# JustinPrivitera/Real_Time_Ray_Tracer

Hardware: AMD Instinct MI355X
Metric: Mrays/s + ms/frame at 3840x2160, 16 AO samples, 64 spheres; 1/2/4/8 GPU (higher is better)
Workload: dtype f32

## Files before the change

__graft_entry__.py:

```python
from __future__ import annotations

import os
import subprocess
import sys
from pathlib import Path

ROOT = Path(__file__).resolve().parent


def build() -> None:
    env = dict(os.environ)
    env.setdefault("PYTORCH_ROCM_ARCH", "gfx950")
    jobs = str(min(16, os.cpu_count() or 1))
    subprocess.run(["make", "-j", jobs, "lib", "headless", "oracle", "b1sort0"], cwd=ROOT, check=True, env=env)
    if str(ROOT) not in sys.path:
        sys.path.insert(0, str(ROOT))
    import real_time_ray_tracer_amd as rt

    rt.load()


def smoke() -> None:
    if str(ROOT) not in sys.path:
        sys.path.insert(0, str(ROOT))
    import numpy as np

    import oracle
    import real_time_ray_tracer_amd as rt

    W, H, spp = 64, 48, 4
    h = rt.Header.synthetic(16, spp, 1234, rt.aspect_for(W, H))
    r = rt.Renderer(W, H, h.S, h.AA, device=0)
    ho = h.copy()
    s = rt.SSBO(ho, W, H)
    d = oracle.dims(W, H, h.S, h.AA)
    img = np.zeros((H, W, 4), np.float32)
    fg = fo = 0
    for k in range(3):
        h.fill_rand_buffer(7000 + k)
        h.set_mode(fg, h.num_objects)
        r.upload_header(h)
        fg = r.dispatch(rt.host._lib.RT_MODE_AO_PP, fg)
        s.set_header(h)
        fo = oracle.dispatch(s.data, d, 1, fo, img)
    g = r.download()
    r.close()
    ok = np.abs(g.image - img) <= 1e-4 * np.maximum(np.abs(g.image), np.abs(img)) + 1e-6
    if not ok.all() or fg != fo:
        raise RuntimeError(f"smoke: {int((~ok).sum())} image values differ from the oracle")
    if not np.array_equal(g.depth.view(np.uint32), s.depth.view(np.uint32)):
        raise RuntimeError("smoke: depth g-buffer differs from the oracle")
    print(f"smoke ok: {W}x{H} mode 1, 3 frames, image mean {img[..., :3].mean():.4f}")


if __name__ == "__main__":
    build()
    if len(sys.argv) > 1 and sys.argv[1] == "smoke":
        smoke()
```

real_time_ray_tracer_amd/csrc/rt_kernels_impl.h:

```cpp
#pragma once
#include <hip/hip_runtime.h>

#include "rt_device.h"
#include "rt_kernels.h"

namespace rt {

namespace {

constexpr int kBlock = 256;
constexpr float kGamma = 1.0f / 2.2f;

__device__ __forceinline__ void stage_shapes(const FrameParams& P, float4* lds) {
  const int n = P.nobj;
  for (int k = threadIdx.x; k < 4 * n; k += blockDim.x) {
    int tab = k / n, i = k - tab * n;
    lds[k] = P.shapes[(size_t)tab * P.S + i];
  }
}

__device__ __forceinline__ f3 primary_dir(const FrameParams& P, float hp, float vp) {
  f3 a = mk(P.lx + hp * P.hx, P.ly + hp * P.hy, P.lz + hp * P.hz);
  return normalize(mk(a.x + vp * P.vx, a.y + vp * P.vy, a.z + vp * P.vz));
}
// ... 506 lines not shown
  float t;
  int ind;
  if (ALLSPH) {
    const ConeF cone = wave_tile_cone<BWX, BWY>(P, bx, by);
    ind = closest_hit_cone<PL>(P, geo, n, cone, cam, dir, 0.0f, t, pre0);
  } else {
    ind = closest_hit<ALLSPH>(geo, geo2, n, cam, dir, 0.0f, t);
  }
  count_work(P, active, y, 1u, active && ind != -1 ? 1u : 0u);
  const bool need = active && ind != -1;
  bool lit_w = true;
  if (ALLSPH) lit_w = shadow_lit_cone<PL>(P, geo, n, light, cam + t * dir, need, pre0);
  if (!active) return;
  float r, g, b;
  if (ind == -1) {
    r = P.bg.x; g = P.bg.y; b = P.bg.z;
  } else {
    f3 curr = cam + t * dir;
    bool lit = ALLSPH ? lit_w : shadow_lit<ALLSPH>(geo, geo2, n, light, curr);
    int id = (ALLSPH && !PL) ? SHAPE_SPHERE : __float_as_int(geo2[ind].w);
    f3 nn = shape_normal(tab[ind], id, curr);
    float4 c = col[ind];
    if (lit) {
      f3 l = normalize(light - curr);
      float spec = pow500(gclamp(dot(normalize(l - dir), nn), 0.0f, 1.0f));
      float k = gclamp(dot(nn, l), 0.06f, 1.0f);
      r = c.x * k + spec; g = c.y * k + spec; b = c.z * k + spec;
    } else {
      r = c.x * 0.06f; g = c.y * 0.06f; b = c.z * 0.06f;
    }
  }
  store_color(P, fd.out_pix, fd.image, x, y, gamma_out(0.0f + r, 0.0f + g, 0.0f + b));
}

#ifndef RT_TAB_LDS_MAX
#define RT_TAB_LDS_MAX 128
#endif
constexpr int kTabLdsMax = RT_TAB_LDS_MAX;
__device__ __forceinline__ void stage_tables(const FrameParams& P, float4* lds) {
  const int n = P.nobj;
  stage_shapes(P, lds);
  for (int k = threadIdx.x; k < n; k += blockDim.x) lds[4 * n + k] = P.sph[k];
}

template <bool ALLSPH, bool PL = false, bool LT = false, bool MF = true>
__global__ __launch_bounds__(kBlock) void phong_kernel(const float4* __restrict__ gsph, const float4* __restrict__ gshp,
                                                       FrameParams P) {
  extern __shared__ float4 lds[];
  if (!ALLSPH || LT) {
    if (LT) stage_tables(P, lds);
    else stage_shapes(P, lds);
    __syncthreads();
  }
  if constexpr (!MF) {
    const float4 g0 = gsph[threadIdx.x & 63];
    phong_tile<ALLSPH, PL, LT>(P, lds, blockIdx.x, blockIdx.y, frame_dst<false>(P, 0), gsph, gshp,
                               (ALLSPH && !LT) ? &g0 : nullptr);
    return;
  }
  int j0;
  const int nj = block_frames<kPhongFramesPerBlock>(P, j0);
#pragma unroll 1
  for (int j = 0; j < nj; ++j)
    phong_tile<ALLSPH, PL, LT>(P, lds, blockIdx.x, blockIdx.y, frame_dst(P, j0 + j), gsph, gshp);
}

template <bool PL>
__device__ __forceinline__ void bounce_round(const FrameParams& P, const float4* __restrict__ geo, int n, f3 light,
                                             bool live, f3 pos, f3 dir, int* perm, float& t_out, int& ind_out,
                                             bool& lit_out) {
  const unsigned long long lm = __ballot(live);
  const int L = __popcll(lm);
  const int lane = threadIdx.x & 63;
  if (L > 32) {
    float t = -1.0f;
    int ind = -1;
    bool lit = true;
    if (live) {
      ind = closest_hit_pf(geo, n, pos, dir, 0.001f, t);
      if (PL) plane_pass(P, pos, dir, 0.001f, t, ind);
      if (ind != -1) lit = shadow_lit_sph<PL>(P, geo, n, light, pos + t * dir);
    }
    t_out = t;
    ind_out = ind;
    lit_out = lit;
    return;
  }
  int c = 0;
  while ((1 << c) < L) ++c;
  const int G = 64 >> c;
  const int rk = __builtin_amdgcn_mbcnt_hi((unsigned)(lm >> 32), __builtin_amdgcn_mbcnt_lo((unsigned)lm, 0u));
  if (live) perm[rk] = lane;
  __builtin_amdgcn_wave_barrier();
  const int g = lane / G, pl = lane - g * G;
  const bool act = g < L;
  const int owner = act ? perm[g] : lane;
  __builtin_amdgcn_wave_barrier();
  const f3 o = mk(__shfl(pos.x, owner), __shfl(pos.y, owner), __shfl(pos.z, owner));
  const f3 d = mk(__shfl(dir.x, owner), __shfl(dir.y, owner), __shfl(dir.z, owner));
  float t = -1.0f;
  int ind = -1;
  if (act)
    for (int i = pl; i < n; i += G) sphere_candidate(o, d, geo[i], i, 0.001f, t, ind);
  for (int m = 1; m < G; m <<= 1) {
    const float tb = __shfl_xor(t, m);
    const int ib = __shfl_xor(ind, m);
    const bool take = ib >= 0 && (ind < 0 || tb < t || (tb == t && ib < ind));
    t = take ? tb : t;
    ind = take ? ib : ind;
  }
  if (PL && act) plane_pass(P, o, d, 0.001f, t, ind);
  bool occ = false;
  if (act && ind != -1) {
    const f3 curr = o + t * d;
    const f3 lv = light - curr;
    const f3 l = normalize(lv);
    const float len = sqrtf(dot(lv, lv));
    const f3 np = curr + 0.01f * l;
    const double dlen = (double)len;
    const ShadowBounds sb = shadow_bounds(l, len);
    if (PL)
      for (int k = pl; k < P.nplanes && !occ; k += G)
        occ = shadow_occludes(plane_eval(np, l, P.planes[2 * k], P.planes[2 * k + 1]), l, dlen, sb);
    for (int i = pl; i < n && !occ; i += G) occ = shadow_occludes(sphere_eval_shadow(np, l, geo[i]), l, dlen, sb);
  }
  unsigned oc = occ ? 1u : 0u;
  for (int m = 1; m < G; m <<= 1) oc |= (unsigned)__shfl_xor((int)oc, m);
  const int src = live ? rk * G : lane;
  t_out = __shfl(t, src);
  ind_out = __shfl(ind, src);
  lit_out = __shfl((int)oc, src) == 0;
}

template <bool ALLSPH, bool PL, bool LT, int ABL = 0, int BWX = 2, int BWY = 2>
__device__ __forceinline__ void hybrid_tile(const FrameParams& P, const float4* lds, int* perm, int bx, int by,
                                            const FrameDst& fd, const float4* __restrict__ gsph,
                                            const float4* __restrict__ gshp, const float4* pre0 = nullptr) {
  const int n = P.nobj;
  const float4* tab = (ALLSPH && !LT) ? gshp : lds;
  const float4* geo = (ALLSPH && !LT) ? gsph : (ALLSPH ? lds + 4 * n : lds);
  const int stride = (ALLSPH && !LT) ? P.S : n;
  const float4 *geo2 = tab + stride, *col = tab + 2 * stride, *aux = tab + 3 * stride;
  int x, y;
  tile_xy<BWX, BWY>(x, y, P.trace_row0, bx, by);
  const bool active = x < P.W && y < P.trace_row0 + P.trace_rows;
  const f3 light = fd.light;
  const unsigned long long tstart = ABL == 7 ? __builtin_amdgcn_s_memrealtime() : 0;
  f3 pos = mk(P.cx, P.cy, P.cz);
  f3 dir = primary_dir(P, div_rn_by((float)x, P.fW, P.inv_W), div_rn_by((float)y, P.fH, P.inv_H));
  float arefl = 0.0f;
  float rr = 0, rg = 0, rb = 0;
  float c = 0.0f;
  unsigned nseg = 0, nshadow = 0;
  auto segment = [&](int seg, float t, int ind, bool lit) -> bool {
    ++nseg;
    nshadow += ind == -1 ? 0u : 1u;
    float ar, ag, ab;
    bool stop;
    if (ind == -1) {
      ar = P.bg.x; ag = P.bg.y; ab = P.bg.z;
      stop = true;
    } else {
      float4 att = ABL == 9 ? make_float4(0.5f, 0.5f, 0.5f, 0.0f) : col[ind];
      f3 curr = pos + t * dir;
      int id = (ALLSPH && !PL) ? SHAPE_SPHERE : __float_as_int(geo2[ind].w);
      f3 nn = ABL == 9 ? normalize(curr) : shape_normal(tab[ind], id, curr);
      if (lit) {
        f3 l = normalize(light - curr);
        float spec = pow500(gclamp(dot(normalize(l - dir), nn), 0.0f, 1.0f));
        float k = gclamp(dot(nn, l), 0.06f, 1.0f);
        ar = att.x * k + spec; ag = att.y * k + spec; ab = att.z * k + spec;
      } else {
        ar = att.x * 0.06f; ag = att.y * 0.06f; ab = att.z * 0.06f;
      }
      float refl = ABL == 9 ? 0.0f : 1.0f - aux[ind].y;
      if (refl < 0.001f) {
        stop = true;
      } else {
        stop = false;
        float dn = dot(dir, nn);
        dir = normalize(mk(dir.x - 2.0f * (dn * nn.x), dir.y - 2.0f * (dn * nn.y),
                           dir.z - 2.0f * (dn * nn.z)));
        pos = curr;
        arefl = refl;
      }
    }
    if (seg == 0) {
      c = arefl;
      rr = ar; rg = ag; rb = ab;
    } else {
      float den = 1.0f + c;
      rr = (rr + c * ar) / den;
      rg = (rg + c * ag) / den;
      rb = (rb + c * ab) / den;
      c = c * arefl;
    }
    return stop;
  };
  if (ALLSPH) {
    float t0 = -1.0f;
    int ind0 = -1;
    bool lit0 = true;
    const ConeF cone = wave_tile_cone<BWX, BWY>(P, bx, by);
    if (ABL != 2) ind0 = closest_hit_cone<PL, ABL == 3>(P, geo, n, cone, pos, dir, 0.001f, t0, pre0);
    if (ABL == 0 || ABL >= 4) lit0 = shadow_lit_cone<PL>(P, geo, n, light, pos + t0 * dir, active && ind0 != -1, pre0);
    bool live = active && !segment(0, t0, ind0, lit0);
    int rounds = 0;
    for (int seg = 1; seg < ((ABL == 5 || ABL == 9) ? 1 : P.D); ++seg) {
      if (__ballot(live) == 0) break;
      ++rounds;
      float t;
      int ind;
      bool lit = true;
      if (ABL == 6) {
        if (live) {
          ind = closest_hit_pf(geo, n, pos, dir, 0.001f, t);
          if (PL) plane_pass(P, pos, dir, 0.001f, t, ind);
          if (ind != -1) lit = shadow_lit_sph<PL>(P, geo, n, light, pos + t * dir);
        }
      } else {
        bounce_round<PL>(P, geo, n, light, live, pos, dir, perm, t, ind, lit);
      }
      if (live) live = !segment(seg, t, ind, lit);
    }
    if (P.tile_cost && (threadIdx.x & 63) == 0)
      P.tile_cost[((unsigned)by * gridDim.x + (unsigned)bx) * (BWX * BWY) + (threadIdx.x >> 6)] = (unsigned)rounds;
  } else {
    for (int seg = 0; active && seg < P.D; ++seg) {
      float t;
      const int ind = closest_hit<ALLSPH>(geo, geo2, n, pos, dir, 0.001f, t);
      const bool lit = ind == -1 || shadow_lit<ALLSPH>(geo, geo2, n, light, pos + t * dir);
      if (segment(seg, t, ind, lit)) break;
    }
  }
  count_work(P, active, y, nseg, nshadow);
  if (active) store_color(P, fd.out_pix, fd.image, x, y, gamma_out(0.0f + rr, 0.0f + rg, 0.0f + rb));
  if (ABL == 7) {
    const unsigned mx = wave_max(active ? nseg : 0u);
    const unsigned long long tend = __builtin_amdgcn_s_memrealtime();
    if ((threadIdx.x & 63) == 0 && active)
      P.out_pix[(size_t)(y - P.band_row0) * P.W + x] =
          make_float4(__uint_as_float((unsigned)tstart), __uint_as_float((unsigned)tend), __uint_as_float(mx),
                      __uint_as_float((unsigned)(tstart >> 32)));
  }
}

template <bool ALLSPH, bool PL = false, bool LT = false, int ABL = 0, int BWX = 2, int BWY = 2, bool MF = true>
__global__ __launch_bounds__(64 * BWX * BWY) void hybrid_kernel(const unsigned* __restrict__ tord,
                                                                const float4* __restrict__ gsph,
                                                                const float4* __restrict__ gshp, unsigned gx,
                                                                FrameParams P) {
  extern __shared__ float4 lds[];
  __shared__ int hperm[64 * BWX * BWY];
  if (!ALLSPH || LT) {
    if (LT) stage_tables(P, lds);
    else stage_shapes(P, lds);
    __syncthreads();
  }
  if constexpr (kHybridTilesPerBlock == 2) {
    const unsigned gx = gridDim.x, gy = (unsigned)(P.trace_rows + 8 * BWY - 1) / (8 * BWY), n = gx * gy;
    const unsigned b = blockIdx.x + blockIdx.y * gx;
#pragma unroll 1
    for (int t = 0; t < 2; ++t) {
      const unsigned u = t == 0 ? b : n - 1 - b;
      if (b > n - 1 - b || (t == 1 && u == b)) break;
      unsigned bx = u % gx, by = u / gx;
      if (tord) {
        const unsigned v = tord[u];
        bx = v & 0xffffu;
        by = v >> 16;
      }
      hybrid_tile<ALLSPH, PL, LT, ABL, BWX, BWY>(P, lds, hperm + 64 * (threadIdx.x >> 6), bx, by, frame_dst(P, blockIdx.z), gsph, gshp);
    }
  } else if constexpr (kHybridTilesPerBlock > 1) {
#pragma unroll 1
    for (int t = 0; t < kHybridTilesPerBlock; ++t)
      hybrid_tile<ALLSPH, PL, LT, ABL, BWX, BWY>(P, lds, hperm + 64 * (threadIdx.x >> 6), blockIdx.x,
                                                 blockIdx.y * kHybridTilesPerBlock + t, frame_dst(P, blockIdx.z), gsph, gshp);
  } else if constexpr (kHybridFramesPerBlock == 1) {
    const bool pre = !MF && ALLSPH && !LT;
    float4 g0;
    if (pre) g0 = gsph[threadIdx.x & 63];
    unsigned bx = blockIdx.x, by = blockIdx.y;
    if (tord) {
      const unsigned t = tord[blockIdx.x + blockIdx.y * gx];
      bx = t & 0xffffu;
      by = t >> 16;
    }
    hybrid_tile<ALLSPH, PL, LT, ABL, BWX, BWY>(P, lds, hperm + 64 * (threadIdx.x >> 6), bx, by,
                                               frame_dst<MF>(P, blockIdx.z), gsph, gshp, pre ? &g0 : nullptr);
  } else {
    int j0;
    const int nj = block_frames<kHybridFramesPerBlock>(P, j0);
#pragma unroll 1
    for (int j = 0; j < nj; ++j)
      hybrid_tile<ALLSPH, PL, LT, ABL, BWX, BWY>(P, lds, hperm + 64 * (threadIdx.x >> 6), blockIdx.x, blockIdx.y,
                                                 frame_dst(P, j0 + j), gsph, gshp);
  }
}

enum { PRIM_HIT = 0, PRIM_MISS = 1, PRIM_EMISSIVE = 2 };

struct BatchLds {
  int prec, sres, pstop, pkind, perm, order, cmask, rls, geol, total;
};
__host__ __device__ constexpr BatchLds batch_lds(int spp, int pool, int ntail, bool rls_lds = true, bool sort = false) {
  const int TP = pool / spp > 0 ? pool / spp : 1, NS = TP * spp;
  BatchLds L{};
  L.prec = 0;
  L.sres = 16 * TP;
  L.pstop = L.sres + 12 * NS;
  L.pkind = L.pstop + 4 * TP;
  L.perm = L.pkind + 4 * ((TP + 1) & ~1);
  L.order = L.perm + 256;
  L.cmask = (L.order + (sort ? pool : 0) + 7) & ~7;
  L.rls = (L.cmask + 8 * 32 + 15) & ~15;
  L.geol = L.rls + (rls_lds ? 32 * spp : 0);
  L.total = L.geol + 16 * ntail;
  return L;
}

#ifndef RT_AO_MINW
#define RT_AO_MINW 7
#endif
#ifndef RT_PT_WIDE
#define RT_PT_WIDE 1
#endif
#ifndef RT_B1_DEFER
#define RT_B1_DEFER 1
#endif
#ifndef RT_B1_PRIO
#define RT_B1_PRIO 1
#endif
#ifndef RT_START_PRIO
#define RT_START_PRIO 1
#endif
#ifndef RT_B1_CREAD
#define RT_B1_CREAD 1
#endif
#ifndef RT_B1_SORT
#define RT_B1_SORT 1
#endif
constexpr int kAoMinWaves = RT_AO_MINW;
template <int MINW, bool LAZY = true, int POOL = kPool, int ABL = 0, bool TAIL = false, bool B1 = false,
          int SPPC = 0, bool PT = false, bool CNT = true, bool PL = false, bool MF = false, bool CL = true, int DC = 0,
          bool CLON = false, bool PTW = false, bool SORT = false>
__global__ __launch_bounds__(64, MINW) void ao_batch_kernel(FrameParams P, const float4* __restrict__ geo) {
  if (RT_START_PRIO) __builtin_amdgcn_s_setprio(1);
  unsigned long long* const cnts = CNT ? P.counters : nullptr;
  unsigned long long* const rowc = CNT ? P.row_counters : nullptr;
  extern __shared__ float4 lds[];
  const int spp = SPPC ? SPPC : P.spp, W = P.W, D = DC ? DC : P.D, nobj = P.nobj;
  const bool use_cl = CL && (CLON || P.ncl > 0);
  const int fj = MF ? (int)blockIdx.y : 0;
  const int fslot = MF ? (P.mf_slot0 + fj) % P.F : 0;
  float4* const f_nrm = MF ? (float4*)P.hist_nrm[fslot] : P.nrm;
  float4* const f_dep = MF ? (float4*)P.hist_dep[fslot] : P.dep;
  const float4* const f_nrm_prev = MF ? f_nrm : P.nrm_prev;
  const float4* const f_dep_prev = MF ? f_dep : P.dep_prev;
  float4* const f_out = MF ? (float4*)P.hist_pix[fslot] : P.out_pix;
  float4* const f_img = MF ? (fj == P.mf_n - 1 ? P.image : nullptr) : P.image;
  const float4* const f_rb = MF ? P.mf_rb + (size_t)fj * 2 * spp : P.rb;
  const int TP = POOL / spp > 0 ? POOL / spp : 1;
  const int lane = threadIdx.x;
  const int NS = TP * spp;
  static_assert(!SORT || (LAZY && POOL % 64 == 0 && POOL <= 256), "SORT: hemi is read back from LDS; items are bytes");
  const BatchLds LO = batch_lds(spp, POOL, 0, !PTW, SORT);
  char* lbase = (char*)lds;
  float4* prec = (float4*)(lbase + LO.prec);
  float* sres = (float*)(lbase + LO.sres);
  int* pstop = (int*)(lbase + LO.pstop);
  int* pkind = (int*)(lbase + LO.pkind);
  int* perm = (int*)(lbase + LO.perm);
  unsigned char* order = (unsigned char*)(lbase + LO.order);
  unsigned long long* cmask = (unsigned long long*)(lbase + LO.cmask);
  float4* rls = (float4*)(lbase + LO.rls);
  if (!PTW)
    for (int k = lane; k < 2 * spp; k += 64) rls[k] = f_rb[k];
  for (int k = lane; k < TP; k += 64) pstop[k] = -1;
  float4* geol = (float4*)(lbase + LO.geol);
  constexpr bool tail_lds = TAIL && PT && !PTW;
  const bool tail_ok = TAIL;
  const float4* const tgeo = tail_lds ? geol : geo;
  const bool pt_ok = PT && B1 && (tail_lds || PTW);
  bool geol_valid = false;
  if (tail_lds && !pt_ok) {
    for (int k = lane; k < nobj; k += 64) geol[k] = geo[k];
    geol_valid = true;
  }
  const float4* const clus = geo + (size_t)3 * P.S;
  const unsigned long long* const clm = (const unsigned long long*)(geo + (size_t)3 * P.S + kMaxClusters);
  auto col_at = [&](int ind) -> float4 {
    int o = ind - P.S;
    asm("" : "+v"(o));
    return geo[o - P.S];
  };
  auto aux_at = [&](int ind) -> float4 {
    int o = ind - P.S;
    asm("" : "+v"(o));
    return geo[o];
  };

  const long long npix = (long long)P.trace_rows * W;
  unsigned pb = blockIdx.x;
  if (P.pool_rot > 0) {
    const unsigned Q = (unsigned)P.pool_rot, r = pb / Q;
    if ((r + 1) * Q <= gridDim.x) {
      unsigned c = pb - r * Q + r % Q;
      c = c >= Q ? c - Q : c;
      pb = r * Q + c;
    }
  }
  const long long p0 = (long long)pb * TP;
  const int np = (int)(npix - p0 < TP ? npix - p0 : TP);
  const int total = np * spp;

  unsigned long long tsec[8] = {0, 0, 0, 0, 0, 0, 0, 0};
  constexpr bool kLaps = ABL == 3 || ABL == 6 || ABL == 8;
  unsigned long long tmark = kLaps ? __builtin_amdgcn_s_memtime() : 0;
  auto lap = [&](int k) {
    if (kLaps) {
      unsigned long long now = __builtin_amdgcn_s_memtime();
      tsec[k] += now - tmark;
      tmark = now;
    }
  };
  const int yf = P.trace_row0 + (int)(p0 / W), xf = (int)(p0 % W);
  auto pool_xy = [&](int lp, int& x, int& y) {
    int xi = xf + lp;
    y = yf;
    if (xi >= W) {
      int q = (int)((unsigned)xi / (unsigned)W);
      y += q;
      xi -= q * W;
    }
    x = xi;
  };
  const int yl = P.trace_row0 + (int)((p0 + np - 1) / W), xl = (int)((p0 + np - 1) % W);
  int ncull = 0;
  const int nwords = (nobj + 63) >> 6;
  unsigned long long pmask = 0;
  {
    const ConeF cone = pool_cone_f(P, yf == yl ? xf : 0, yf == yl ? xl : W - 1, yf, yl);
    for (int w = 0; w < nwords; ++w) {
      int i = (w << 6) + lane;
      bool keep = i < nobj && !cone_misses_f(cone, geo[i], P.cx, P.cy, P.cz);
      if (PL) keep = keep && geo[i].x == geo[i].x;
      unsigned long long m = __ballot(keep);
      ncull += __popcll(m);
      if (lane == 0) cmask[w] = m;
    }
    if (PL) {
      pmask = plane_cone_mask(P, cone, mk(P.cx, P.cy, P.cz));
      ncull += __popcll(pmask) + (P.nplanes > 64 ? P.nplanes - 64 : 0);
    }
  }
  __syncthreads();
  lap(0);
  if (RT_START_PRIO) __builtin_amdgcn_s_setprio(0);

  if (LAZY && ncull == 0) {
    const float fa = (float)spp;
    float sr = 0.0f, sg = 0.0f, sb = 0.0f;
    for (int k = 0; k < spp; ++k) {
      sr = sr + 1.0f * P.bg.x; sg = sg + 1.0f * P.bg.y; sb = sb + 1.0f * P.bg.z;
    }
    const float4 col = gamma_out(sr / fa, sg / fa, sb / fa);
    const float4 z = make_float4(0.0f, 0.0f, 0.0f, 0.0f);
    for (int lp = lane; lp < np; lp += 64) {
      int x, y;
      pool_xy(lp, x, y);
      const size_t off = (size_t)(y - P.band_row0) * W + x;
      nrm_store(f_nrm, dep_plane(P), off, z);
      dep_store(f_dep, dep_plane(P), off, z);
      store_color(P, f_out, f_img, x, y, col);
      if (rowc) atomicAdd(&rowc[y - P.band_row0], (unsigned long long)spp);
    }
    if (cnts && lane == 0 && ABL < 3) {
      unsigned long long* c = cnts + (blockIdx.x & (kCounterSlots - 1));
      atomicAdd(&c[0 * kCounterSlots], (unsigned long long)total);
      atomicAdd(&c[1 * kCounterSlots], (unsigned long long)total);
      atomicAdd(&c[3 * kCounterSlots], (unsigned long long)total * (unsigned long long)nobj);
    }
    return;
  }

  const f3 cam = mk(P.cx, P.cy, P.cz);
  const float4* rbuf = PTW ? f_rb : rls;
  bool has = false;
  int item = 0, depth = 0;
  f3 pos = cam, dir = cam, hemi = cam;
  float rr = 1.0f, rg = 1.0f, rb = 1.0f;
  int bitem = 0;
  f3 bpos = cam, bdir = cam, bhemi = cam;
  float br = 1.0f, bg = 1.0f, bb = 1.0f;
  int next = 0, cursor = 0, nlive = 0, bdepth = D - 1;
  int b1cost = nobj;
  unsigned nseg = 0;
  unsigned long long exec_tests = 0;

  const float inv_spp = P.inv_spp;
  auto div_spp = [&](int it) { return SPPC ? (int)((unsigned)it / (unsigned)SPPC) : (int)(((float)it + 0.5f) * inv_spp); };
  auto finish = [&](int it, float r, float g, float b, float stopv, int segs) {
    sres[it] = r;
    sres[NS + it] = g;
    sres[2 * NS + it] = b;
    if (stopv >= 0.0f) {
      const int lq = div_spp(it);
      atomicMax(&pstop[lq], ((it - lq * spp) << 16) | (int)stopv);
    }
    if (rowc) {
      int x, y;
      pool_xy(div_spp(it), x, y);
      atomicAdd(&rowc[y - P.band_row0],
                (unsigned long long)(kSetupCost + ncull + (segs >= 2 ? b1cost + (segs - 2) * nobj : 0)));
    }
  };

  auto shade = [&](int ind, float t, f3& ps, f3& dr, f3 hm, float& r, float& g, float& b, int dpt, int it,
                   bool first) -> bool {
    const int lp = div_spp(it), aa = it - lp * spp;
    float4 att = col_at(ind);
    int kind = PRIM_MISS;
    bool go = false;
    if (ind != -1) {
      const float4 ax = aux_at(ind);
      float4 gc = make_float4(0.0f, 0.0f, 0.0f, 0.0f);
      if (!PL) {
        gc = geo[ind];
        asm volatile("" ::"v"(gc.x), "v"(gc.y), "v"(gc.z));
      }
      if (ax.x > 0.9f) {
        kind = PRIM_EMISSIVE;
      } else {
        kind = PRIM_HIT;
        f3 curr = cam + t * dr;
        f3 nn;
        if (PL) {
          const float4 gi = P.shapes[ind];
          nn = __float_as_int(P.shapes[P.S + ind].w) == SHAPE_PLANE ? xyz(gi) : normalize(curr - xyz(gi));
        } else {
          nn = normalize(curr - xyz(gc));
        }
        if (aa == 0 && first) prec[lp] = make_float4(nn.x, nn.y, nn.z, t);
        if (ABL == 9) {
          float z;
          asm volatile("v_mov_b32 %0, 0" : "=v"(z));
          const f3 c2 = cam + (t + z) * dr;
          const f3 n2 = normalize(c2 - (PL ? xyz(P.shapes[ind]) : xyz(gc)));
          const float d2 = dot(dr, n2);
          const f3 R2 = normalize(mk(dr.x - 2.0f * (d2 * n2.x), dr.y - 2.0f * (d2 * n2.y), dr.z - 2.0f * (d2 * n2.z)));
          const f3 X2 = normalize(ax.y > 0.999f ? hm + n2 : R2 + ax.y * hm);
          if (__float_as_uint(X2.x + X2.y + X2.z) == 0x7fc00001u) t = X2.x;
        }
        ps = curr;
        const float reflect = ax.y;
        f3 X;
        if (reflect > 0.999f) {
          X = hm + nn;
        } else {
          float dn = dot(dr, nn);
          f3 R = normalize(mk(dr.x - 2.0f * (dn * nn.x), dr.y - 2.0f * (dn * nn.y), dr.z - 2.0f * (dn * nn.z)));
          X = R + reflect * hm;
        }
        dr = normalize(X);
        go = dpt - 1 != 0;
      }
    }
    r = r * att.x; g = g * att.y; b = b * att.z;
    if (aa == 0 && first) pkind[lp] = kind;
    if (!go) finish(it, r, g, b, kind == PRIM_HIT ? -1.0f : (float)(D - dpt), kind == PRIM_HIT ? D : D - dpt + 1);
    return go;
  };

  auto prepare = [&]() {
    bitem = next + lane;
    bool live = false;
    if (ABL == 3) { tsec[6] += (unsigned long long)ncull; tsec[7] += 1; }
    exec_tests += (unsigned long long)ncull;
    if (bitem < total) {
      if (SORT) bitem = order[bitem];
      const int lp = div_spp(bitem), aa = bitem - lp * spp;
      int x, y;
      pool_xy(lp, x, y);
      const float px = (float)x, py = (float)y;
      float hp, vp;
      {
        float4 f = rbuf[2 * aa], s = rbuf[2 * aa + 1];
        float uw[2];
        grandom_n<2>({((s.x + px * f.z) - px) + f.x, s.z * px - (f.x * px) * f.z},
                     {((f.y + py * s.w) - py) + s.y, f.w * py - (s.y * py) * s.w}, uw);
        if (ABL == 4) {
          float z, uw2[2];
          asm volatile("v_mov_b32 %0, 0" : "=v"(z));
          grandom_n<2>({((s.x + px * f.z) - px) + f.x + z, s.z * px - (f.x * px) * f.z + z},
                       {((f.y + py * s.w) - py) + s.y, f.w * py - (s.y * py) * s.w}, uw2);
          if (__float_as_uint(uw2[0]) == 0x7fc00001u && __float_as_uint(uw2[1]) == 0x7fc00001u) uw[0] = uw2[0];
        }
        float u = uw[0], w = uw[1];
        normalize2(u, w);
        const float jx = aa == 0 ? 0.0f : div_rn_by(u, 6.0f, kInv6) - 0.08333f;
        const float jy = aa == 0 ? 0.0f : div_rn_by(w, 6.0f, kInv6) - 0.08333f;
        hp = div_rn_by(px + jx, P.fW, P.inv_W);
        vp = div_rn_by(py + jy, P.fH, P.inv_H);
      }
      bdir = primary_dir(P, hp, vp);
      if (ABL == 10) {
        float z;
        asm volatile("v_mov_b32 %0, 0" : "=v"(z));
        float u2 = hp + z, w2 = vp + z;
        normalize2(u2, w2);
        const float jx2 = aa == 0 ? 0.0f : div_rn_by(u2, 6.0f, kInv6) - 0.08333f;
        const float jy2 = aa == 0 ? 0.0f : div_rn_by(w2, 6.0f, kInv6) - 0.08333f;
        const f3 d2 = primary_dir(P, div_rn_by(px + jx2, P.fW, P.inv_W), div_rn_by(py + jy2, P.fH, P.inv_H));
        if (__float_as_uint(d2.x + d2.y + d2.z) == 0x7fc00001u) bdir.x = d2.y;
      }
      auto hemisphere = [&]() {
        float4 f = rbuf[2 * aa], s = rbuf[2 * aa + 1];
        float abe[3];
        grandom_n<3>({f.x + px * s.z, f.z - px * s.z, s.x * px + s.z}, {f.y + py * s.w, f.w - py * s.w, s.y * py + s.w},
                     abe);
        if (ABL == 4) {
          float z, abe2[3];
          asm volatile("v_mov_b32 %0, 0" : "=v"(z));
          grandom_n<3>({f.x + px * s.z + z, f.z - px * s.z + z, s.x * px + s.z + z},
                       {f.y + py * s.w, f.w - py * s.w, s.y * py + s.w}, abe2);
          if (__float_as_uint(abe2[0]) == 0x7fc00001u && __float_as_uint(abe2[2]) == 0x7fc00001u) abe[1] = abe2[1];
        }
        return normalize(mk(abe[0] * 2.0f - 1.0f, abe[1] * 2.0f - 1.0f, abe[2] * 2.0f - 1.0f));
      };
      if (!LAZY) bhemi = hemisphere();
      f3 cv = cam;
      asm("" : "+v"(cv.x), "+v"(cv.y), "+v"(cv.z));
      bpos = cv;
      br = bg = bb = 1.0f;
      float t = -1.0f;
      int ind = -1;
      for (int w = 0; w < nwords; ++w) {
        unsigned long long m = cmask[w];
        m = ((unsigned long long)__builtin_amdgcn_readfirstlane((unsigned)(m >> 32)) << 32) |
            (unsigned)__builtin_amdgcn_readfirstlane((unsigned)m);
        const float4* const gw = geo + (w << 6);
        while (m) {
          const unsigned j = (unsigned)pop_lowest(m);
          const int i = (w << 6) + (int)j;
          sphere_candidate(bpos, bdir, gw[j], i, 0.0001f, t, ind);
          if (ABL == 2) {
            float z;
            asm volatile("v_mov_b32 %0, 0" : "=v"(z));
            float t2 = -1.0f;
            int i2 = -1;
            sphere_candidate(mk(bpos.x + z, bpos.y, bpos.z), bdir, geo[i], i, 0.0001f, t2, i2);
            if (i2 == 0x7fffffff) t = t2;
          }
        }
      }
      if (PL) plane_pass_masked(P, pmask, bpos, bdir, 0.0001f, t, ind);
      ++nseg;
      if (LAZY && ind != -1) bhemi = SORT ? mk(sres[bitem], sres[NS + bitem], sres[2 * NS + bitem]) : hemisphere();
      live = shade(ind, t, bpos, bdir, bhemi, br, bg, bb, D, bitem, true);
    }
    bdepth = D - 1;
    b1cost = nobj;
    if (B1) {
      const unsigned long long lm1 = __ballot(live);
      if (lm1 != 0 && __popcll(lm1) >= P.b1_min) {
        lap(1);
        if (RT_B1_PRIO) __builtin_amdgcn_s_setprio(1);
        const ConeB cb = bounce_cone(live, bpos, bdir, lm1);
        float t = -1.0f;
        int ind = -1;
        b1cost = 0;
        if (ABL == 12) {
          float z;
          asm volatile("v_mov_b32 %0, 0" : "=v"(z));
          const ConeB c2 = bounce_cone(live, mk(bpos.x + z, bpos.y, bpos.z), bdir, lm1);
          unsigned long long acc = 0;
          for (int w = 0; w < nwords; ++w) {
            const int i = (w << 6) + lane_id_here();
            float4 pt;
            const bool k2 = i < nobj && bounce_cone_keep_pt(c2, geo[i], pt);
            acc ^= __ballot(k2 && pt.w != 7.0f);
          }
          if (acc == 0x123456789abcdefull) b1cost = 1;
        }
        unsigned long long ru = 0;
        int ksel = 0;
        f3 tdir = bdir;
        if (RT_B1_DEFER && !live) tdir = mk(__int_as_float(0x7fc00000), __int_as_float(0x7fc00000), __int_as_float(0x7fc00000));
        auto flush = [&]() {
          const float4 gs = geo[ksel];
          sphere_candidate_if(bpos, bdir, gs, ksel, 0.0001f, t, ind, ru);
          ru = 0;
        };
        for (int w = 0; w < nwords; ++w) {
          const int i = (w << 6) + lane_id_here();
          bool keep;
          if (pt_ok) {
            float4 pt;
            keep = i < nobj && bounce_cone_keep_pt(cb, geo[i], pt);
            if (i < nobj) geol[PTW ? i - (w << 6) : i] = pt;
          } else {
            keep = i < nobj && !bounce_cone_misses(cb, geo[i]);
          }
          if (PL) keep = keep && geo[i].x == geo[i].x;
          unsigned long long m = __ballot(keep);
          m = ((unsigned long long)__builtin_amdgcn_readfirstlane((unsigned)(m >> 32)) << 32) |
              (unsigned)__builtin_amdgcn_readfirstlane((unsigned)m);
          exec_tests += (unsigned long long)__popcll(m);
          b1cost += __popcll(m);
          if (ABL == 3) tsec[6] += (unsigned long long)__popcll(m) << 24;
          if (pt_ok) {
            geol_valid = false;
            __syncthreads();
            if (ABL == 6) lap(5);
            const float4* const qw = geol + (PTW ? 0 : (w << 6));
            const float4* const gw = geo + (w << 6);
            int qbase;
            asm("v_mov_b32 %0, %1" : "=v"(qbase) : "s"((int)(size_t)((const char*)qw - lbase)));
            if (RT_B1_DEFER || live)
              while (m) {
                const int j = pop_lowest(m), k = (w << 6) + j;
#if RT_B1_CREAD
                const float4 q = *(const float4*)(lbase + (qbase + (j << 4)));
#else
                typedef float v4f __attribute__((ext_vector_type(4)));
                v4f qv;
                int j_addr_scratch;
                asm volatile("v_lshl_add_u32 %1, %2, 4, %3\n\tds_read_b128 %0, %1\n\ts_waitcnt lgkmcnt(0)"
                             : "=v"(qv), "=&v"(j_addr_scratch)
                             : "s"(j), "v"(qbase));
                const float4 q = make_float4(qv.x, qv.y, qv.z, qv.w);
#endif
                const float4 g = gw[j];
                if (ABL == 7) {
                  const bool pass = fmaf(bdir.z, q.z, fmaf(bdir.y, q.y, bdir.x * q.x)) >= q.w;
                  const f3 pmc = bpos - xyz(g);
                  const float bb = dot(bdir, pmc);
                  const float del = fmaf(g.w, g.w, fmaf(bb, bb, -dot(pmc, pmc)));
                  const unsigned long long pm = __ballot(pass), dm = __ballot(pass && del >= 0.0f);
                  tsec[0] += 1; tsec[1] += pm != 0; tsec[2] += dm != 0;
                  tsec[3] += (unsigned long long)__popcll(pm);
                }
                const bool pass = fmaf(tdir.z, q.z, fmaf(tdir.y, q.y, tdir.x * q.x)) >= q.w;
                if (ABL == 5) {
                  float z, t2 = t;
                  int i2 = ind;
                  asm volatile("v_mov_b32 %0, 0" : "=v"(z));
                  const bool pass2 = fmaf(bdir.z + z, q.z, fmaf(bdir.y, q.y, bdir.x * q.x)) >= q.w;
                  const unsigned long long pm2 = __builtin_amdgcn_ballot_w64(pass2);
                  if (pm2 != 0) sphere_candidate_if(mk(bpos.x + z, bpos.y, bpos.z), bdir, g, k, 0.0001f, t2, i2, pm2);
                  if (i2 == 0x7fffffff) t = t2;
                }
                const unsigned long long pm = __builtin_amdgcn_ballot_w64(pass);
                if (RT_B1_DEFER) {
                  if (pm != 0) {
                    if (pm & ru) flush();
                    ru |= pm;
                    int kv = k;
                    asm("v_cndmask_b32_e64 %0, %1, %2, %3" : "=v"(ksel) : "v"(ksel), "v"(kv), "s"(pm));
                  }
                } else if (pm != 0) {
                  sphere_candidate_if(bpos, bdir, g, k, 0.0001f, t, ind, pm);
                }
              }
            if (ABL == 6) lap(6);
          } else if (live) {
            while (m) {
              const int k = (w << 6) + __builtin_ctzll(m);
              m &= m - 1;
              sphere_candidate(bpos, bdir, geo[k], k, 0.0001f, t, ind);
            }
          }
        }
        if (RT_B1_DEFER && ru != 0) flush();
        if (RT_B1_PRIO) __builtin_amdgcn_s_setprio(0);
        if (ABL == 7) { tsec[4] += 1; tsec[5] += (unsigned long long)__popcll(lm1); }
        if (live) {
          if (PL) plane_pass(P, bpos, bdir, 0.0001f, t, ind);
          ++nseg;
          live = shade(ind, t, bpos, bdir, bhemi, br, bg, bb, D - 1, bitem, false);
        }
        if (ABL == 6) lap(7);
        bdepth = D - 2;
        lap(4);
      }
    }
    unsigned long long lm = __ballot(live);
    if (live) perm[__builtin_amdgcn_mbcnt_hi((unsigned)(lm >> 32), __builtin_amdgcn_mbcnt_lo((unsigned)lm, 0u))] = lane;
    nlive = __popcll(lm);
    cursor = 0;
    next = next + 64 < total ? next + 64 : total;
    __syncthreads();
  };

  if (SORT) {
    constexpr int NC = POOL / 64, NF = 3;
    static_assert(NC * (1 << NF) <= 64, "one cell per lane");
    const int ln = lane_id_here();
    perm[ln] = 0;
    __syncthreads();
    int key[NC];
#pragma unroll
    for (int c = 0; c < NC; ++c) {
      key[c] = 0;
      if (c * 64 < total) {
        const int it = c * 64 + ln;
        f3 h = mk(0.0f, 0.0f, 0.0f);
        if (it < total) {
          const int lp = div_spp(it), aa = it - lp * spp;
          int x, y;
          pool_xy(lp, x, y);
          const float px = (float)x, py = (float)y;
          const float4 f = rbuf[2 * aa], s = rbuf[2 * aa + 1];
          float abe[3];
          grandom_n<3>({f.x + px * s.z, f.z - px * s.z, s.x * px + s.z}, {f.y + py * s.w, f.w - py * s.w, s.y * py + s.w},
                       abe);
          h = normalize(mk(abe[0] * 2.0f - 1.0f, abe[1] * 2.0f - 1.0f, abe[2] * 2.0f - 1.0f));
          sres[it] = h.x;
          sres[NS + it] = h.y;
          sres[2 * NS + it] = h.z;
        }
        const int nv = total - c * 64;
        const unsigned long long mv = nv >= 64 ? ~0ull : (1ull << nv) - 1;
        unsigned own_lo = (unsigned)mv, own_hi = (unsigned)(mv >> 32);
        unsigned oct = 0;
        const float hc[NF] = {h.x, h.y, h.z};
#pragma unroll
        for (int k = NF - 1; k >= 0; --k) {
          const int bits = __float_as_int(hc[k]);
          const unsigned long long m = __ballot(bits < 0);
          const unsigned sgn = (unsigned)(bits >> 31);
          own_lo &= ~((unsigned)m ^ sgn);
          own_hi &= ~((unsigned)(m >> 32) ^ sgn);
          oct = oct << 1 | (unsigned)bits >> 31;
        }
        const int cell = (int)oct * NC + c;
        const int r = (int)__builtin_amdgcn_mbcnt_hi(own_hi, __builtin_amdgcn_mbcnt_lo(own_lo, 0u));
        if (it < total) perm[cell] = __popc(own_lo) + __popc(own_hi);
        key[c] = r | cell << 8;
      }
    }
    __syncthreads();
    {
      const int bin = ln / NC, c = ln % NC;
      const bool in = ln < NC * (1 << NF);
      const int cell = in ? (bin ^ (bin >> 1)) * NC + c : 0;
      const int n = in ? perm[cell] : 0;
      int acc = n;
      acc += __builtin_amdgcn_update_dpp(0, acc, 0x111, 0xf, 0xf, false);
      acc += __builtin_amdgcn_update_dpp(0, acc, 0x112, 0xf, 0xf, false);
      acc += __builtin_amdgcn_update_dpp(0, acc, 0x114, 0xf, 0xf, false);
      acc += __builtin_amdgcn_update_dpp(0, acc, 0x118, 0xf, 0xf, false);
      acc += __builtin_amdgcn_update_dpp(0, acc, 0x142, 0xa, 0xf, false);
      acc += __builtin_amdgcn_update_dpp(0, acc, 0x143, 0xc, 0xf, false);
      __syncthreads();
      if (in) perm[cell] = acc - n;
    }
    __syncthreads();
#pragma unroll
    for (int c = 0; c < NC; ++c) {
      const int it = c * 64 + ln;
      if (it < total) order[perm[key[c] >> 8] + (key[c] & 255)] = (unsigned char)it;
    }
    __syncthreads();
  }

  for (;;) {
    for (;;) {
      unsigned long long need = __ballot(!has);
      if (need == 0) break;
      if (cursor >= nlive) {
        if (next >= total) break;
        lap(2);
        prepare();
        lap(1);
        continue;
      }
      int r = __builtin_amdgcn_mbcnt_hi((unsigned)(need >> 32), __builtin_amdgcn_mbcnt_lo((unsigned)need, 0u));
      int take = __popcll(need) < nlive - cursor ? __popcll(need) : nlive - cursor;
      bool get = !has && r < take;
      int src = get ? perm[cursor + r] : lane;
      float sx = __shfl(bpos.x, src), sy = __shfl(bpos.y, src), sz = __shfl(bpos.z, src);
      float dx = __shfl(bdir.x, src), dy = __shfl(bdir.y, src), dz = __shfl(bdir.z, src);
      float hx = __shfl(bhemi.x, src), hy = __shfl(bhemi.y, src), hz = __shfl(bhemi.z, src);
      float cr = __shfl(br, src), cg = __shfl(bg, src), cb = __shfl(bb, src);
      int ci = __shfl(bitem, src);
      if (ABL == 11) {
        int zi;
        asm volatile("v_mov_b32 %0, 0" : "=v"(zi));
        const int s2 = src + zi;
        float q = __shfl(bpos.x, s2) + __shfl(bpos.y, s2) + __shfl(bpos.z, s2) + __shfl(bdir.x, s2) + __shfl(bdir.y, s2) +
                  __shfl(bdir.z, s2) + __shfl(bhemi.x, s2) + __shfl(bhemi.y, s2) + __shfl(bhemi.z, s2) + __shfl(br, s2) +
                  __shfl(bg, s2) + __shfl(bb, s2) + (float)__shfl(bitem, s2);
        if (__float_as_uint(q) == 0x7fc00001u) cr = q;
      }
      if (get) {
        pos = mk(sx, sy, sz);
        dir = mk(dx, dy, dz);
        hemi = mk(hx, hy, hz);
        rr = cr; rg = cg; rb = cb;
        item = ci;
        depth = bdepth;
        has = true;
      }
      cursor += take;
    }
    const unsigned long long hm = __ballot(has);
    if (hm == 0) break;
    lap(2);
    if (ABL == 3) tsec[5] += 1;
    const int L = __popcll(hm);
    if (tail_ok && next >= total && cursor >= nlive && L <= 32) {
      if (tail_lds && !geol_valid) {
        __syncthreads();
        for (int k = lane_id_here(); k < nobj; k += 64) geol[k] = geo[k];
        geol_valid = true;
      }
      int c = 0;
      while ((1 << c) < L) ++c;
      const int G = 64 >> c;
      const int rk = __builtin_amdgcn_mbcnt_hi((unsigned)(hm >> 32), __builtin_amdgcn_mbcnt_lo((unsigned)hm, 0u));
      if (has) perm[rk] = lane;
      __syncthreads();
      const int g = lane / G, pl = lane - g * G;
      const bool act = g < L;
      const int owner = act ? perm[g] : lane;
      const f3 o = mk(__shfl(pos.x, owner), __shfl(pos.y, owner), __shfl(pos.z, owner));
      const f3 d = mk(__shfl(dir.x, owner), __shfl(dir.y, owner), __shfl(dir.z, owner));
      float t = -1.0f;
      int ind = -1;
      if (use_cl && G <= kClusterTailMaxG) {
        unsigned long long kc = 0;
        for (int c0 = 0; c0 < P.ncl; c0 += G) {
          const int c = c0 + pl;
          const bool may = act && c < P.ncl && cluster_may_hit(o, d, clus[c]);
          unsigned long long b = __builtin_amdgcn_ballot_w64(may);
          for (int sh = 32; sh >= G; sh >>= 1) b |= b >> sh;
          kc |= (G == 64 ? b : (b & ((1ull << G) - 1))) << c0;
        }
        unsigned char* list = (unsigned char*)cmask;
        int cnt = 0;
        for (int w = 0; w < nwords; ++w) {
          unsigned long long m = clm[w];
          for (unsigned long long k2 = kc; k2;) m |= clm[(size_t)(1 + pop_lowest(k2)) * kClusterWords + w];
          const int ln = lane_id_here();
          if ((m >> ln) & 1ull)
            list[cnt + __builtin_amdgcn_mbcnt_hi((unsigned)(m >> 32), __builtin_amdgcn_mbcnt_lo((unsigned)m, 0u))] =
                (unsigned char)((w << 6) + ln);
          cnt += __popcll(m);
        }
        __syncthreads();
        exec_tests += (unsigned long long)((P.ncl + G - 1) / G + (cnt + G - 1) / G);
        if (act) {
          int i = list[pl < cnt ? pl : 0];
          for (int k = pl; k < cnt; k += G) {
            const float4 g = tgeo[i];
            const int inext = list[k + G < cnt ? k + G : cnt - 1];
            sphere_candidate(o, d, g, i, 0.0001f, t, ind);
            i = inext;
          }
        }
      } else if (act) {
        for (int i = pl; i < nobj; i += G) sphere_candidate(o, d, tgeo[i], i, 0.0001f, t, ind);
      }
      for (int m = 1; m < G; m <<= 1) {
        const float tb = __shfl_xor(t, m);
        const int ib = __shfl_xor(ind, m);
        const bool take = ib >= 0 && (ind < 0 || tb < t || (tb == t && ib < ind));
        t = take ? tb : t;
        ind = take ? ib : ind;
      }
      float tt = __shfl(t, rk * G);
      int ii = __shfl(ind, rk * G);
      if (!(use_cl && G <= kClusterTailMaxG)) exec_tests += (unsigned long long)((nobj + G - 1) / G);
      if (has) {
        if (PL) plane_pass(P, pos, dir, 0.0001f, tt, ii);
        ++nseg;
        has = shade(ii, tt, pos, dir, hemi, rr, rg, rb, depth, item, false);
        depth -= 1;
      }
      if (ABL == 8) tsec[7] += 1;
      lap(ABL == 8 ? 5 : 3);
      continue;
    }
    exec_tests += (unsigned long long)(use_cl ? P.ncl : nobj);
    if (ABL == 7) {
      tsec[6] += (unsigned long long)nobj;
      for (int i = 0; i < nobj; ++i) {
        const float4 g = geo[i];
        const f3 pmc = pos - xyz(g);
        const float bb = dot(dir, pmc);
        const float del = fmaf(g.w, g.w, fmaf(bb, bb, -dot(pmc, pmc)));
        tsec[7] += __ballot(has && del >= 0.0f) != 0;
      }
    }
    if (use_cl) {
      unsigned long long kc = 0;
      for (int c = 0; c < P.ncl; c += 4) {
        const float4 c0 = clus[c], c1 = clus[c + 1], c2 = clus[c + 2], c3 = clus[c + 3];
#if RT_CL_MASKS
        const unsigned long long b0 = cluster_may_hit_mask(pos, dir, c0) & hm;
        const unsigned long long b1 = cluster_may_hit_mask(pos, dir, c1) & hm;
        const unsigned long long b2 = cluster_may_hit_mask(pos, dir, c2) & hm;
        const unsigned long long b3 = cluster_may_hit_mask(pos, dir, c3) & hm;
        unsigned nib = (b0 ? 16u : 0u) | (b1 ? 32u : 0u) | (b2 ? 64u : 0u) | (b3 ? 128u : 0u);
        asm("" : "+s"(nib));
        kc |= (unsigned long long)(nib >> 4) << c;
#else
        const unsigned long long b0 = __builtin_amdgcn_ballot_w64(cluster_may_hit(pos, dir, c0)) & hm;
        const unsigned long long b1 = __builtin_amdgcn_ballot_w64(cluster_may_hit(pos, dir, c1)) & hm;
        const unsigned long long b2 = __builtin_amdgcn_ballot_w64(cluster_may_hit(pos, dir, c2)) & hm;
        const unsigned long long b3 = __builtin_amdgcn_ballot_w64(cluster_may_hit(pos, dir, c3)) & hm;
        kc |= (unsigned long long)((b0 != 0) | (b1 != 0) << 1 | (b2 != 0) << 2 | (b3 != 0) << 3) << c;
#endif
// ... 567 lines not shown
```

Baseline: 63910.

## Compact bounce-cone survivors into LDS rows and unroll the candidate test loop

Instead of storing every object's cone-test data in LDS and then walking the ballot mask bit by bit, surviving candidates are written into a dense compacted LDS array, ordered by rank from mbcnt. The object index is packed into the low mantissa bits of the threshold, with an optional separate index table. The consumer loop then processes U rows per iteration with no bit scanning, and padding rows make overrun rows fail. The aim is to cut the serial pop-lowest and LDS address overhead in the first-bounce loop, at the cost of a slightly perturbed threshold, extra LDS padding and more complex code.

```diff
diff --git a/__graft_entry__.py b/__graft_entry__.py
--- a/__graft_entry__.py
+++ b/__graft_entry__.py
@@ -12,7 +12,7 @@
     env = dict(os.environ)
     env.setdefault("PYTORCH_ROCM_ARCH", "gfx950")
     jobs = str(min(16, os.cpu_count() or 1))
-    subprocess.run(["make", "-j", jobs, "lib", "headless", "oracle", "b1sort0"], cwd=ROOT, check=True, env=env)
+    subprocess.run(["make", "-j", jobs, "lib", "headless", "oracle", "b1sort0", "b1compact0"], cwd=ROOT, check=True, env=env)
     if str(ROOT) not in sys.path:
         sys.path.insert(0, str(ROOT))
     import real_time_ray_tracer_amd as rt
diff --git a/real_time_ray_tracer_amd/csrc/rt_kernels_impl.h b/real_time_ray_tracer_amd/csrc/rt_kernels_impl.h
--- a/real_time_ray_tracer_amd/csrc/rt_kernels_impl.h
+++ b/real_time_ray_tracer_amd/csrc/rt_kernels_impl.h
@@ -832,8 +832,24 @@
 enum { PRIM_HIT = 0, PRIM_MISS = 1, PRIM_EMISSIVE = 2 };
 
 struct BatchLds {
-  int prec, sres, pstop, pkind, perm, order, cmask, rls, geol, total;
+  int prec, sres, pstop, pkind, perm, order, cmask, rls, kidx, geol, total;
 };
+#ifndef RT_B1_COMPACT
+#define RT_B1_COMPACT 1
+#endif
+#ifndef RT_B1_COMPACT_U
+#define RT_B1_COMPACT_U 4
+#endif
+#ifndef RT_B1_COMPACT_KIDX
+#define RT_B1_COMPACT_KIDX 0
+#endif
+#ifndef RT_B1_COMPACT_AHEAD
+#define RT_B1_COMPACT_AHEAD 0
+#endif
+#ifndef RT_B1_COMPACT_ALL
+#define RT_B1_COMPACT_ALL 0
+#endif
+constexpr int kB1PadRows = RT_B1_COMPACT ? RT_B1_COMPACT_U - 1 : 0;
 __host__ __device__ constexpr BatchLds batch_lds(int spp, int pool, int ntail, bool rls_lds = true, bool sort = false) {
   const int TP = pool / spp > 0 ? pool / spp : 1, NS = TP * spp;
   BatchLds L{};
@@ -845,8 +861,9 @@
   L.order = L.perm + 256;
   L.cmask = (L.order + (sort ? pool : 0) + 7) & ~7;
   L.rls = (L.cmask + 8 * 32 + 15) & ~15;
-  L.geol = L.rls + (rls_lds ? 32 * spp : 0);
-  L.total = L.geol + 16 * ntail;
+  L.kidx = L.rls + (rls_lds ? 32 * spp : 0);
+  L.geol = L.kidx + (RT_B1_COMPACT && RT_B1_COMPACT_KIDX ? 128 : 0);
+  L.total = L.geol + 16 * (ntail + (ntail > 0 ? kB1PadRows : 0));
   return L;
 }
 
@@ -905,6 +922,8 @@
   unsigned char* order = (unsigned char*)(lbase + LO.order);
   unsigned long long* cmask = (unsigned long long*)(lbase + LO.cmask);
   float4* rls = (float4*)(lbase + LO.rls);
+  unsigned short* kidx = (unsigned short*)(lbase + LO.kidx);
+  constexpr bool COMPACT = RT_B1_COMPACT && (PTW || PL || RT_B1_COMPACT_ALL) && ABL != 5 && ABL != 7;
   if (!PTW)
     for (int k = lane; k < 2 * spp; k += 64) rls[k] = f_rb[k];
   for (int k = lane; k < TP; k += 64) pstop[k] = -1;
@@ -1226,10 +1245,10 @@
         for (int w = 0; w < nwords; ++w) {
           const int i = (w << 6) + lane_id_here();
           bool keep;
+          float4 pt;
           if (pt_ok) {
-            float4 pt;
             keep = i < nobj && bounce_cone_keep_pt(cb, geo[i], pt);
-            if (i < nobj) geol[PTW ? i - (w << 6) : i] = pt;
+            if (!COMPACT && i < nobj) geol[PTW ? i - (w << 6) : i] = pt;
           } else {
             keep = i < nobj && !bounce_cone_misses(cb, geo[i]);
           }
@@ -1240,7 +1259,67 @@
           exec_tests += (unsigned long long)__popcll(m);
           b1cost += __popcll(m);
           if (ABL == 3) tsec[6] += (unsigned long long)__popcll(m) << 24;
-          if (pt_ok) {
+          if (pt_ok && COMPACT) {
+            geol_valid = false;
+            constexpr int U = RT_B1_COMPACT_U;
+            const int n = __popcll(m);
+            float4* const qw = geol + (PTW ? 0 : (w << 6));
+            const float4* const gw = geo + (w << 6);
+            if (n != 0) {
+              const int ln = lane_id_here();
+              const int rank = (int)__builtin_amdgcn_mbcnt_hi((unsigned)(m >> 32), __builtin_amdgcn_mbcnt_lo((unsigned)m, 0u));
+              if (RT_B1_COMPACT_KIDX && keep) kidx[rank] = (unsigned short)((w << 6) + ln);
+              const float kp = RT_B1_COMPACT_KIDX ? pt.w : __uint_as_float((__float_as_uint(pt.w - 4e-5f) & ~63u) | (unsigned)ln);
+              const float4 row = make_float4(keep ? pt.x : 0.0f, keep ? pt.y : 0.0f, keep ? pt.z : 0.0f, keep ? kp : 2.0f);
+              const int slot = keep ? rank : n + ln - rank;
+              if ((w << 6) + ln < nobj + (U - 1)) qw[slot] = row;
+            }
+            __syncthreads();
+            if (ABL == 6) lap(5);
+            int qa;
+            typedef float v4f __attribute__((ext_vector_type(4)));
+            typedef const __attribute__((address_space(3))) v4f* lds_row_ptr;
+            asm("v_mov_b32 %0, %1" : "=v"(qa) : "s"((int)(size_t)(lds_row_ptr)(const v4f*)qw));
+            if (RT_B1_DEFER || live) {
+#pragma unroll 1
+              for (int r = 0; r < n; r += U) {
+#if RT_B1_COMPACT_AHEAD
+                v4f qrow[U];
+#pragma unroll
+                for (int u = 0; u < U; ++u) qrow[u] = *(lds_row_ptr)(size_t)(unsigned)(qa + 16 * u);
+#endif
+#pragma unroll
+                for (int u = 0; u < U; ++u) {
+#if RT_B1_COMPACT_AHEAD
+                  const v4f q = qrow[u];
+#else
+                  const v4f q = *(lds_row_ptr)(size_t)(unsigned)(qa + 16 * u);
+#endif
+                  const bool pass = fmaf(tdir.z, q.z, fmaf(tdir.y, q.y, tdir.x * q.x)) >= q.w;
+                  const unsigned long long pm = __builtin_amdgcn_ballot_w64(pass);
+                  if (pm != 0) {
+                    float kw = q.w;
+                    if (RT_B1_DEFER && (pm & ru)) {
+                      flush();
+                      if (!RT_B1_COMPACT_KIDX)
+                        kw = *(volatile const __attribute__((address_space(3))) float*)(size_t)(unsigned)(qa + 16 * u + 12);
+                    }
+                    int kv = RT_B1_COMPACT_KIDX ? (int)kidx[r + u] : (int)((__float_as_uint(kw) & 63u) | (unsigned)(w << 6));
+                    if (RT_B1_DEFER) {
+                      ru |= pm;
+                      asm("v_cndmask_b32_e64 %0, %1, %2, %3" : "=v"(ksel) : "v"(ksel), "v"(kv), "s"(pm));
+                    } else {
+                      const int k = __builtin_amdgcn_readfirstlane(kv);
+                      sphere_candidate_if(bpos, bdir, gw[k - (w << 6)], k, 0.0001f, t, ind, pm);
+                    }
+                  }
+                }
+                qa += 16 * U;
+                asm("" : "+v"(qa));
+              }
+            }
+            if (ABL == 6) lap(6);
+          } else if (pt_ok) {
             geol_valid = false;
             __syncthreads();
             if (ABL == 6) lap(5);
```

Result: no change. 64000, median of 6 (+0.1%).
